# Lu-Zhan/Pano-NeRF

Hardware: AMD Instinct MI355X
Metric: rays/sec (train step) (higher is better)
Workload: dtype f32 (2xfp16 split products, fp32 accumulate; weight-gradient operands h_l / delta_l / r_l / hdot_l stored with 16 significant bits, 'Q24')

## Files before the change

### pano-nerf_amd/csrc/pn_chain.hip

```cpp
#include "pn_common.h"
#include <math.h>
#include <string.h>
#include <stdlib.h>
#include <type_traits>
#include <utility>
#include <vector>

template <typename F, int... Is>
__device__ __forceinline__ void static_for_impl(F&& f, std::integer_sequence<int, Is...>) {
    (f(std::integral_constant<int, Is>{}), ...);
}
template <int N, typename F>
__device__ __forceinline__ void static_for(F&& f) {
    static_for_impl(static_cast<F&&>(f), std::make_integer_sequence<int, N>{});
}

typedef __bf16 bf16x8 __attribute__((ext_vector_type(8)));
typedef _Float16 f16x8 __attribute__((ext_vector_type(8)));
typedef __attribute__((address_space(3))) void* lds_ptr_t;
typedef const __attribute__((address_space(1))) void* gbl_ptr_t;

#ifndef PN_CHAIN_TILE
#define PN_CHAIN_TILE 16
#endif
// ... 153 lines not shown
    constexpr int CF = Cfg<NP>::CF, SLOT = Cfg<NP>::SLOT, PER = Cfg<NP>::PER;
    const int64_t gid = (int64_t)blockIdx.x * blockDim.x + threadIdx.x;
    const int lane = (int)(gid & 63);
    const int64_t fi = gid >> 6;
    const int chunk = (int)(fi / (CF + 1)), f = (int)(fi % (CF + 1));
    if (chunk >= tab.nchunks) return;
    int li = 0;
    for (int i = 1; i < tab.n; ++i)
        if (chunk >= tab.L[i].chunk0) li = i;
    const PackLayer& L = tab.L[li];
    unsigned char* dst = out + (int64_t)chunk * SLOT + f * 1024 + lane * 16;
    if (f == CF) {
        float v[4] = {0.f, 0.f, 0.f, 0.f};
        if (chunk == L.chunk0 + (L.KS * L.NT + PER - 1) / PER - 1 && L.aux_off >= 0)
            for (int q = 0; q < 4; ++q)
                if (lane * 4 + q < L.aux_n) v[q] = params[L.aux_off + lane * 4 + q];
        memcpy(dst, v, 16);
        return;
    }
    const int p = f % NP;
    const int step = (chunk - L.chunk0) * PER + f / NP;
    int wex = 0;
    if constexpr (NP == 2) {
        const uint32_t* wm = reinterpret_cast<const uint32_t*>(wexp) + 32 + li * WEXP_SLICES;
        uint32_t top = 0u;
#pragma unroll
        for (int sl = 0; sl < WEXP_SLICES; ++sl) top = wm[sl] > top ? wm[sl] : top;
        wex = scale_exp(__uint_as_float(top), EXP_CAP_W);
        if (chunk == L.chunk0 && f == 0 && lane == 0) wexp[li] = wex;
    }
    unsigned short o[8] = {0, 0, 0, 0, 0, 0, 0, 0};
    if (step < L.KS * L.NT) {
        const int ks = step / L.NT, tt = step % L.NT;
        const int i = TILE * tt + (lane % TILE), g = lane / TILE;
        for (int j = 0; j < 8; ++j) {
            const int k = kmap(ks, g, j);
            float x = 0.f;
            if (i < L.rows_valid)
                for (int s = 0; s < L.nseg; ++s) {
                    const PackSeg& sg = L.seg[s];
                    const int kr = k - sg.k0;
                    if (kr >= 0 && kr < sg.kvalid)
                        x = sg.transposed ? params[sg.off + (int64_t)kr * sg.ld + sg.col0 + i]
                                          : params[sg.off + (int64_t)i * sg.ld + sg.col0 + kr];
                }
            unsigned short bits;
            if constexpr (NP == 2) {
                const float t = ldexpf(x, wex);
                const _Float16 hh = (_Float16)t;
                const _Float16 r = p == 0 ? hh : (_Float16)(t - (float)hh);
                __builtin_memcpy(&bits, &r, 2);
            } else {
                const __bf16 hb = (__bf16)x;
                __bf16 r = hb;
                if (p >= 1) {
                    const float r1 = x - (float)hb;
                    const __bf16 mb = (__bf16)r1;
                    r = mb;
                    if (p == 2) r = (__bf16)(r1 - (float)mb);
                }
                __builtin_memcpy(&bits, &r, 2);
            }
            o[j] = bits;
        }
    }
    memcpy(dst, o, 16);
}

#if defined(PN_TRACE_CHAIN) || defined(PN_TRACE_WG)
__device__ unsigned long long g_chain_trace[64];
extern "C" int pn_chain_trace_read(unsigned long long* out) {
    return hipMemcpyFromSymbol(out, HIP_SYMBOL(g_chain_trace), sizeof(unsigned long long) * 64) == hipSuccess ? 0 : -4;
}
#endif
#ifdef PN_TRACE_CHAIN
#define TR(i)                                                                                          \
    do {                                                                                               \
        if (blockIdx.x == 0 && threadIdx.x == 0 && st == (int64_t)gridDim.x) g_chain_trace[i] = __builtin_amdgcn_s_memtime(); \
    } while (0)
#define TRX(i)                                                                                 \
    do {                                                                                       \
        if (blockIdx.x == 0 && threadIdx.x == 0) g_chain_trace[i] = __builtin_amdgcn_s_memtime(); \
    } while (0)
#else
#define TR(i)
#define TRX(i)
#endif

template <int NP>
struct Ring {
    static constexpr int CF = Cfg<NP>::CF, SLOT = Cfg<NP>::SLOT;
    static constexpr int PIECES = CF / CH_WAVES + 1;
    __amdgpu_buffer_rsrc_t rsrc;
    unsigned char* lds;
    uint32_t lds_addr;
    int nchunk;
    int pf, pslot, cslot;
    int wid, lane;
    int cur_soff;
    unsigned char* cur_lds;
    __device__ __forceinline__ void begin_round() {
        cur_soff = pf * SLOT;
        cur_lds = lds + pslot * SLOT;
        pf = (pf + 1 == nchunk) ? 0 : pf + 1;
        pslot = (pslot + 1 == Cfg<NP>::NSLOT) ? 0 : pslot + 1;
    }
    template <int I, bool AUX>
    __device__ __forceinline__ void piece() {
        if constexpr (I < CF / CH_WAVES) {
            const int f = wid + CH_WAVES * I;
            __builtin_amdgcn_raw_ptr_buffer_load_lds(rsrc, (lds_ptr_t)(cur_lds + f * 1024), 16, lane * 16, cur_soff + f * 1024, 0, 0);
        } else if constexpr (I == CF / CH_WAVES && AUX) {
            if (wid < 4) {
                const int o = CF * 1024 + wid * 256;
                __builtin_amdgcn_raw_ptr_buffer_load_lds(rsrc, (lds_ptr_t)(cur_lds + o), 4, lane * 4, cur_soff + o, 0, 0);
            }
        }
    }
    template <int I0, int STRIDE, bool AUX = true>
    __device__ __forceinline__ void pieces_from() {
        if constexpr (I0 < PIECES) {
            piece<I0, AUX>();
            pieces_from<I0 + STRIDE, STRIDE, AUX>();
        }
    }
    __device__ __forceinline__ void start(const unsigned char* s, unsigned char* l, int n, int w, int ln, int first) {
        rsrc = __builtin_amdgcn_make_buffer_rsrc((void*)s, 0, n * SLOT, 0x00020000);
        lds = l; nchunk = n; wid = w; lane = ln;
        lds_addr = (uint32_t)(uintptr_t)(lds_ptr_t)l;
        pf = first; pslot = 0; cslot = 0;
#pragma unroll
        for (int i = 0; i < Cfg<NP>::D; ++i) {
            begin_round();
            pieces_from<0, 1, true>();
        }
    }
#ifdef PN_TRACE_CHAIN
    unsigned long long t_lds = 0, t_dma = 0, t_bar = 0, n_acq = 0;
#endif
    __device__ __forceinline__ uint32_t acquire() {
        constexpr int N = Cfg<NP>::SHARE * (Cfg<NP>::D - 1);
#ifdef PN_TRACE_CHAIN
        const unsigned long long t0 = __builtin_amdgcn_s_memtime();
        asm volatile("s_waitcnt lgkmcnt(0)" ::: "memory");
        const unsigned long long t1 = __builtin_amdgcn_s_memtime();
        asm volatile("s_waitcnt vmcnt(%0) lgkmcnt(0)" ::"n"(N) : "memory");
        const unsigned long long t2 = __builtin_amdgcn_s_memtime();
        __builtin_amdgcn_s_barrier();
        const unsigned long long t3 = __builtin_amdgcn_s_memtime();
        asm volatile("s_waitcnt lgkmcnt(0)" ::: "memory");
        t_lds += t1 - t0; t_dma += t2 - t1; t_bar += t3 - t2; ++n_acq;
#else
        asm volatile("s_waitcnt vmcnt(%0) lgkmcnt(0)" ::"n"(N) : "memory");
        if constexpr (!(PN_ABL_CHAIN & 8)) __builtin_amdgcn_s_barrier();
#endif
        begin_round();
        const uint32_t p = lds_addr + cslot * SLOT;
        cslot = (cslot + 1 == Cfg<NP>::NSLOT) ? 0 : cslot + 1;
        return p;
    }
    __device__ __forceinline__ void drain() {
        asm volatile("s_waitcnt vmcnt(0)" ::: "memory");
        __builtin_amdgcn_s_barrier();
#ifdef PN_TRACE_CHAIN
        if (blockIdx.x == 0 && threadIdx.x == 0) {
            g_chain_trace[56] = t_lds; g_chain_trace[57] = t_dma; g_chain_trace[58] = t_bar; g_chain_trace[59] = n_acq;
        }
#endif
    }
// ... 558 lines not shown
__device__ __forceinline__ Tile tile_of(int64_t st, int wid, int lane, int64_t M) {
    Tile t;
    t.c = lane % TILE;
    t.g = lane / TILE;
    t.blk = st * CH_WAVES + wid;
    t.row = t.blk * TILE + t.c;
    t.live = t.row < M;
    t.rc = t.live ? t.row : M - 1;
    t.lo = t.c + 4 * t.g * TILE;
    return t;
}
template <int NP, int NT>
__device__ __forceinline__ void store_vec(typename TEl<NP>::type* slot, const Tile& T, int F, bool q, const accv (&acc)[NT]) {
    if constexpr (kQ24<NP>) {
        if (q) {
            store_q24<NT>(reinterpret_cast<unsigned char*>(slot) + T.blk * (int64_t)(F * TILE * 3) + opaque(q24_lane(T.c, T.g)), acc);
            return;
        }
    }
    store_t<NT>(slot + T.blk * (int64_t)(F * TILE) + opaque(T.lo), acc);
}

template <int NP, int MODE>
__device__ __forceinline__ Ex encode(const float (&mu)[3], const float (&cv)[3], const float (&vv)[3], int g,
                                      typename TEl<NP>::type* et, BFrag<NP> (&benc)[KS_ENC]) {
    typedef typename TEl<NP>::type TE;
    constexpr int NQ = 96 / QB;
    float x[NQ][4];
    const int g4 = 4 * opaque(g);
#pragma unroll
    for (int qb = 0; qb < NQ / 2; ++qb)
#pragma unroll
        for (int i = 0; i < 4; ++i) {
            int l, ch;
            level_of(QB * qb + g4 + i, l, ch);
            const float sc = pow2i(l);
            const float y = sel3(mu, ch) * sc;
            const float e0 = __expf(-0.5f * (sel3(cv, ch) * (sc * sc)));
            if constexpr (MODE == 0) {
                x[qb][i] = e0 * fast_sin(y);
                x[qb + NQ / 2][i] = e0 * fast_sin(y + HALF_PI_F);
            } else {
                const float e = e0 * sc * sel3(vv, ch);
                x[qb][i] = e * fast_cos(y);
                x[qb + NQ / 2][i] = e * fast_cos(y + HALF_PI_F);
            }
        }
#ifdef PN_TRACE_CHAIN
#pragma unroll
    for (int qb = 0; qb < NQ; ++qb)
#pragma unroll
        for (int i = 0; i < 4; ++i) asm volatile("" ::"v"(x[qb][i]));
    if (MODE == 0) TRX(31);
#endif
#pragma unroll
    for (int qb = 0; qb < NQ; ++qb)
#pragma unroll
        for (int i = 0; i < 4; ++i) et[(QB * qb + i) * TILE] = (TE)x[qb][i];
    if (MODE == 0) TRX(32);
    Ex e{0, 0u};
    if constexpr (NP == 2) {
        if constexpr (MODE == 0) {
            e.ex = EXP_TOP - 1;
            e.top = 0x3f800000u;
        } else {
            float m = 0.f;
#pragma unroll
            for (int qb = 0; qb < NQ; ++qb)
#pragma unroll
                for (int i = 0; i < 4; ++i) m = fmaxf(m, fabsf(x[qb][i]));
            e = ex_of(m, EXP_CAP_Z);
        }
    }
#pragma unroll
    for (int s = 0; s < KS_ENC; ++s) {
        float y8[8];
#pragma unroll
        for (int j = 0; j < 8; ++j) y8[j] = x[2 * s + (j >> 2)][j & 3];
        split_into<NP>(y8, benc[s], e.ex);
    }
    return e;
}
template <int NP, int KS>
__device__ __forceinline__ int reload_b(const typename TEl<NP>::type* src, BFrag<NP> (&b)[KS], int cap = EXP_CAP) {
    if constexpr (NP == 2) {
        float x[KS][8];
        float m = 0.f;
#pragma unroll
        for (int ks = 0; ks < KS; ++ks)
#pragma unroll
            for (int j = 0; j < 8; ++j) {
                x[ks][j] = (float)src[(QB * (2 * ks + (j >> 2)) + (j & 3)) * TILE];
                m = fmaxf(m, fabsf(x[ks][j]));
            }
        const int ex = scale_exp(col_max(m), cap);
#pragma unroll
        for (int ks = 0; ks < KS; ++ks) split_into<NP>(x[ks], b[ks], ex);
        return ex;
    } else {
#pragma unroll
        for (int ks = 0; ks < KS; ++ks) {
            float x[8];
#pragma unroll
            for (int j = 0; j < 8; ++j) x[j] = (float)src[(QB * (2 * ks + (j >> 2)) + (j & 3)) * TILE];
            split_into<NP>(x, b[ks]);
        }
        return 0;
    }
}
__device__ __forceinline__ void ipe_backward_tiles(const accv (&acc)[NT_ENC], const float (&mu)[3], const float (&cv)[3], int g,
                                                   float (&dm)[3]) {
    dm[0] = dm[1] = dm[2] = 0.f;
    const int g4 = 4 * opaque(g);
#pragma unroll
    for (int qb = 0; qb < 96 / QB; ++qb)
#pragma unroll
        for (int i = 0; i < 4; ++i) {
            const bool cosine = qb >= 96 / QB / 2;
            int l, ch;
            level_of(QB * (cosine ? qb - 96 / QB / 2 : qb) + g4 + i, l, ch);
            const float sc = pow2i(l);
            const float y = sel3(mu, ch) * sc;
            const float ex = __expf(-0.5f * (sel3(cv, ch) * (sc * sc))) * sc;
            const float d = AQ(acc, qb, i) * ex * fast_cos(cosine ? y + HALF_PI_F : y);
            dm[0] += ch == 0 ? d : 0.f;
            dm[1] += ch == 1 ? d : 0.f;
            dm[2] += ch == 2 ? d : 0.f;
        }
#pragma unroll
    for (int i = 0; i < 3; ++i) {
        dm[i] = col_sum(dm[i]);
    }
}
template <int NP>
__device__ __forceinline__ Ex finish_gated(accv (&acc)[NT_H], const Gate& m, typename TEl<NP>::type* slot, const Tile& T, bool q24,
                                           BFrag<NP> (&bh)[KS_H]) {
    gate_bits<NT_H>(acc, m);
    if (slot) store_vec<NP, NT_H>(slot, T, 256, q24, acc);
    return acc_to_b<NP, NT_H, KS_H>(acc, bh, 0.f, EXP_CAP_Z);
}

__global__ void k_view_table(int64_t view_rows, const float* viewdirs, float* tab, uint32_t* amax, int amax_n) {
    if (amax && blockIdx.x == 0 && (int)threadIdx.x < amax_n) amax[threadIdx.x] = 0u;
    const int64_t idx = (int64_t)blockIdx.x * blockDim.x + threadIdx.x;
    if (idx >= view_rows * 32) return;
    const int64_t r = idx >> 5;
    const int v = (int)(idx & 31);
    const float vd0 = viewdirs[r * 3], vd1 = viewdirs[r * 3 + 1], vd2 = viewdirs[r * 3 + 2];
    auto vsel = [&](int ch) { return ch == 0 ? vd0 : (ch == 1 ? vd1 : vd2); };
    const int i = v - 3, half = i >= 12 ? 1 : 0;
    int l, ch;
    level_of(i < 0 ? 0 : i - 12 * half, l, ch);
    const float xb = vsel(ch) * pow2i(l & 3);
    const float sv = fast_sin(half ? xb + HALF_PI_F : xb);
    tab[idx] = v < 3 ? vsel(v) : (v < PN_VIEW_DIM ? sv : 0.f);
}

struct FwdArgs {
    int64_t M, nst;
    int rows_per_ray, nc;
    int64_t view_rows;
    const unsigned char* pack;
    const int* wexp;
    uint32_t* amax;
    const float* mean;
    const float* cov;
    const float* viewdirs;
    float* view_tab;
    float* enc_t;
    float* acts_t;
    uint32_t* masks;
    float* raw_rgb;
    float* raw_den;
    int q24;
};
__host__ __device__ constexpr int64_t act_off(int slot, int64_t Mp) {
    return slot <= 8 ? (int64_t)slot * Mp * 256 : 8 * Mp * 256 + Mp * 288;
}
__host__ __device__ constexpr int64_t acts_floats(int64_t Mp) { return 8 * Mp * 256 + Mp * 288 + Mp * 128; }

template <int NP>
__global__ __launch_bounds__(CH_THREADS, CH_MIN_WAVES) void k_chain_fwd(FwdArgs a) {
    extern __shared__ __attribute__((aligned(16))) unsigned char lds[];
    typedef typename TEl<NP>::type TE;
    const int tid = threadIdx.x, lane = tid & 63;
    const int wid = __builtin_amdgcn_readfirstlane(tid >> 6);
    const int64_t Mp = a.nst * CH_SAMPLES;
    chain_prio(wid);
    Ring<NP> R;
    R.start(a.pack, lds, fwd_chunk0<NP>(F_COUNT), wid, lane, 0);
    RunMax<10> RM;
    RM.clear();
#ifdef PN_TRACE_CHAIN
    if (blockIdx.x == 0 && threadIdx.x == 0) {
        g_chain_trace[60] = __builtin_amdgcn_s_memtime();
        g_chain_trace[61] = __builtin_amdgcn_s_memrealtime();
    }
#endif
    int wtab = 0;
    if constexpr (NP == 2) wtab = a.wexp[lane & 15];
    for (int64_t st = blockIdx.x; st < a.nst; st += gridDim.x) {
        const Tile T = tile_of(st, wid, lane, a.M);
        TR(0);
        TE* et = TP(a.enc_t) + T.blk * (96 * TILE) + T.lo;
        BFrag<NP> bh[KS_H];
        accv acc[NT_H];
        Gate mw;
        int bex = 0;
        auto wx = [&](int i) {
            if constexpr (NP == 2) return __builtin_amdgcn_readlane(wtab, i);
            else return 0;
        };
        {
            float mu[3], cv[3];
            const float zero3[3] = {0.f, 0.f, 0.f};
#pragma unroll
            for (int i = 0; i < 3; ++i) {
                mu[i] = a.mean[T.rc * 3 + i];
                cv[i] = a.cov[T.rc * 3 + i];
            }
            BFrag<NP> benc[KS_ENC];
#ifdef PN_TRACE_CHAIN
            asm volatile("" ::"v"(mu[0]), "v"(mu[1]), "v"(mu[2]), "v"(cv[0]), "v"(cv[1]), "v"(cv[2]));
            TRX(30);
#endif
            bex = encode<NP, 0>(mu, cv, zero3, T.g, et, benc).ex;
            TR(1);
            chain_gemm<NP, KS_ENC, NT_H, true, true, true>(R, benc, acc, lane, wx(F_L0) + bex);
            TR(2);
        }
        auto finish_hidden = [&](int slot) {
            relu<NT_H>(acc);
            if (TP(a.acts_t)) store_vec<NP, NT_H>(TP(a.acts_t) + act_off(slot, Mp), T, 256, a.q24 && q24_act(slot), acc);
            const Ex e = acc_to_b<NP, NT_H, KS_H>(acc, bh);
            gate_words<NP, KS_H, KS_H>(bh, mw);
            store_gate(a.masks, slot, Mp, T.blk * TILE + T.c, T.g, mw);
            bex = e.ex;
            RM.upd(slot, e.top);
        };
        finish_hidden(0);
        TR(3);
#pragma unroll 1
        for (int l = 1; l <= 4; ++l) {
            chain_gemm<NP, KS_H, NT_H, true, true, true>(R, bh, acc, lane, wx(F_L0 + l) + bex);
            TR(2 + 2 * l);
            finish_hidden(l);
            TR(3 + 2 * l);
        }
        {
            chain_gemm<NP, KS_H, NT_H, false, true, true>(R, bh, acc, lane, wx(F_L5) + bex);
            BFrag<NP> benc[KS_ENC];
            const int eex = reload_b<NP, KS_ENC>(et, benc);
            chain_gemm<NP, KS_ENC, NT_H, true, false, true>(R, benc, acc, lane, wx(F_L5E) + eex);
            TR(12);
            finish_hidden(5);
            TR(13);
        }
#pragma unroll 1
        for (int l = 6; l <= 7; ++l) {
            chain_gemm<NP, KS_H, NT_H, true, true, true>(R, bh, acc, lane, wx(F_L6 + l - 6) + bex);
            TR(2 + 2 * l);
            finish_hidden(l);
            TR(3 + 2 * l);
        }
        {
            accv ad[1];
            chain_gemm<NP, KS_H, 1, true, true, true>(R, bh, ad, lane, wx(F_DEN) + bex);
            if (T.live) {
#pragma unroll
                for (int i = 0; i < 4; ++i) {
                    const int ch = 4 * T.g + i;
                    if (ch < a.nc) a.raw_den[T.row * a.nc + ch] = ad[0][i];
                }
            }
        }
        TR(18);
        BFrag<NP> bv[KS_H + KS_PAD];
        int vex;
        {
            chain_gemm<NP, KS_H, NT_H, true, true, true>(R, bh, acc, lane, wx(F_EXTRA) + bex);
            TR(19);
            TE* bt = a.acts_t ? TP(a.acts_t) + act_off(8, Mp) + T.blk * (288 * TILE) + T.lo : nullptr;
            if (bt) store_t<NT_H>(bt, acc);
            const Ex e = acc_to_b<NP, NT_H, KS_H + KS_PAD>(acc, bv, 1.0f);
            vex = e.ex;
            RM.upd(8, e.top);
            const float* vt = a.view_tab + ((T.rc / a.rows_per_ray) % a.view_rows) * 32 + 4 * T.g;
#pragma unroll
            for (int q = 0; q < KS_PAD; ++q) {
                float x[8];
#pragma unroll
                for (int h = 0; h < 2; ++h) {
                    const f32x4 v = *reinterpret_cast<const f32x4*>(vt + QB * (2 * q + h));
#pragma unroll
                    for (int i = 0; i < 4; ++i) {
                        x[4 * h + i] = v[i];
                        if (bt) bt[(256 + QB * (2 * q + h) + i) * TILE] = (TE)v[i];
                    }
                }
                split_into<NP>(x, bv[KS_H + q], vex);
            }
        }
        TR(20);
        BFrag<NP> bc[KS_C];
        int cex;
        {
            accv av[NT_C];
            chain_gemm<NP, KS_H + KS_PAD, NT_C, true, true, true>(R, bv, av, lane, wx(F_VIEW) + vex);
            TR(21);
            Gate w4;
            relu<NT_C>(av);
            if (TP(a.acts_t)) store_t<NT_C>(TP(a.acts_t) + act_off(9, Mp) + T.blk * (128 * TILE) + T.lo, av);
            const Ex e = acc_to_b<NP, NT_C, KS_C>(av, bc);
            gate_words<NP, KS_C, KS_C>(bc, w4);
            store_gate(a.masks, 8, Mp, T.blk * TILE + T.c, T.g, w4);
            cex = e.ex;
            RM.upd(9, e.top);
        }
        TR(22);
        {
            accv ac[1];
            chain_gemm<NP, KS_C, 1, true, true, true>(R, bc, ac, lane, wx(F_COLOR) + cex);
            TR(23);
            if (T.live && T.g == 0) {
#pragma unroll
                for (int e = 0; e < 3; ++e) a.raw_rgb[T.row * 3 + e] = ac[0][e];
            }
        }
        TR(24);
    }
    R.drain();
#ifdef PN_TRACE_CHAIN
    if (blockIdx.x == 0 && threadIdx.x == 0) {
        g_chain_trace[62] = __builtin_amdgcn_s_memtime();
        g_chain_trace[63] = __builtin_amdgcn_s_memrealtime();
    }
#endif
    if constexpr (NP == 2) {
        RM.flush(a.amax ? a.amax + AM_ACT0 : nullptr, lane, wid, lds);
        if (a.amax && blockIdx.x == 0 && tid == 0) a.amax[AM_ENC] = 0x3f800000u;
    }
}

struct SweepArgs {
    int64_t M, nst;
    int nc;
    float density_bias;
    const unsigned char* pack;
    int nchunk;
    const int* wexp;
    uint32_t* amax;
    const uint32_t* masks;
    const float* raw_den;
    const float* mean;
    const float* cov;
    const float* wd0;
    const float* v;
    float* vec_t;
    int keep_all;
    float* edot_t;
    float* out3;
    float* sdot;
    int q24;
};

template <int NP>
__global__ __launch_bounds__(CH_THREADS, CH_MIN_WAVES) void k_chain_dgrad(SweepArgs a) {
    extern __shared__ __attribute__((aligned(16))) unsigned char lds[];
    typedef typename TEl<NP>::type TE;
    const int tid = threadIdx.x, lane = tid & 63;
    const int wid = __builtin_amdgcn_readfirstlane(tid >> 6);
    const int64_t Mp = a.nst * CH_SAMPLES;
    chain_prio(wid);
    Ring<NP> R;
    R.start(a.pack, lds, a.nchunk, wid, lane, 0);
    RunMax<8> RM;
    RM.clear();
    int wtab = 0;
    if constexpr (NP == 2) wtab = a.wexp[lane & 15];
    for (int64_t st = blockIdx.x; st < a.nst; st += gridDim.x) {
        const Tile T = tile_of(st, wid, lane, a.M);
        Gate mk[8];
#pragma unroll
        for (int l = 0; l < 8; ++l) mk[l] = load_gate(a.masks, 7 - l, Mp, T.blk * TILE + T.c, T.g);
        float mu[3], cv[3];
#pragma unroll
        for (int i = 0; i < 3; ++i) {
            mu[i] = a.mean[T.rc * 3 + i];
            cv[i] = a.cov[T.rc * 3 + i];
        }
        const float sgm = T.live ? ch_sp_d1(a.raw_den[T.rc * a.nc] + a.density_bias) : 0.f;
        BFrag<NP> bh[KS_H];
        int bex = 0;
        auto wx = [&](int i) {
            if constexpr (NP == 2) return __builtin_amdgcn_readlane(wtab, i);
            else return 0;
        };
        {
            const bool Q7 = kQ24<NP> && a.q24 && q24_delta(7);
            TE* rt = (a.keep_all && !Q7) ? TP(a.vec_t) + (int64_t)7 * Mp * 256 + T.blk * (256 * TILE) + T.lo : nullptr;
            unsigned char* rq = (a.keep_all && Q7) ? reinterpret_cast<unsigned char*>(TP(a.vec_t) + (int64_t)7 * Mp * 256) +
                                                         T.blk * (int64_t)(256 * TILE * 3) + q24_lane(T.c, T.g)
                                                   : nullptr;
            const Gate m7 = pop_front(mk);
            if constexpr (NP == 2) {
                float wm = 0.f;
#pragma unroll
                for (int qb = 0; qb < NT_H * ACCQ; ++qb) {
                    const f32x4 wv = *reinterpret_cast<const f32x4*>(a.wd0 + QB * qb + 4 * T.g);
                    wm = fmaxf(fmaxf(wm, fmaxf(fabsf(wv[0]), fabsf(wv[1]))), fmaxf(fabsf(wv[2]), fabsf(wv[3])));
                }
                const Ex e = ex_of(sgm * wm, EXP_CAP_Z);
                bex = e.ex;
                RM.upd(7, e.top);
            }
#pragma unroll
            for (int ks = 0; ks < KS_H; ++ks) {
                float x[8];
#pragma unroll
                for (int h = 0; h < 2; ++h) {
                    const f32x4 wv = *reinterpret_cast<const f32x4*>(a.wd0 + QB * (2 * ks + h) + 4 * T.g);
#pragma unroll
                    for (int i = 0; i < 4; ++i) {
                        const int j = 4 * h + i;
                        const uint32_t bit = (m7.w[gate_word(ks, j)] >> gate_bit(ks, j)) & 1u;
                        x[j] = bit ? sgm * wv[i] : 0.f;
                        if (rt) rt[(QB * (2 * ks + h) + i) * TILE] = (TE)x[j];
                    }
                    if constexpr (kQ24<NP>) {
                        if (rq) {
#if PN_Q24_NT
                            __builtin_nontemporal_store(pack_q24(x[4 * h], x[4 * h + 1], x[4 * h + 2], x[4 * h + 3]), reinterpret_cast<u32x3*>(rq + (2 * ks + h) * 768));
#else
                            *reinterpret_cast<u32x3*>(rq + (2 * ks + h) * 768) = pack_q24(x[4 * h], x[4 * h + 1], x[4 * h + 2], x[4 * h + 3]);
#endif
                        }
                    }
                }
                split_into<NP>(x, bh[ks], bex);
            }
        }
        accv acc[NT_H];
#pragma unroll 1
        for (int l = 7; l >= 1; --l) {
            chain_gemm<NP, KS_H, NT_H, false, true>(R, bh, acc, lane, wx(B_L7 + 7 - l) + bex);
            TE* dst = a.keep_all ? TP(a.vec_t) + (int64_t)(l - 1) * Mp * 256 : (l - 1 == 5 ? TP(a.vec_t) : nullptr);
            const Ex e = finish_gated<NP>(acc, pop_front(mk), dst, T, a.q24 && q24_delta(l - 1), bh);
            bex = e.ex;
            RM.upd(l - 1, e.top);
        }
        {
            accv a3[NT_ENC];
            chain_gemm<NP, KS_H, NT_ENC, false, true>(R, bh, a3, lane, wx(B_DENC0) + bex);
            bex = reload_b<NP, KS_H>(TP(a.vec_t) + (a.keep_all ? (int64_t)5 * Mp * 256 : 0) + T.blk * (256 * TILE) + T.lo, bh, EXP_CAP_Z);
            chain_gemm<NP, KS_H, NT_ENC, false, false>(R, bh, a3, lane, wx(B_DENC1) + bex);
            float dm[3];
            ipe_backward_tiles(a3, mu, cv, T.g, dm);
            if (T.live && T.g == 0) {
                a.out3[T.row * 3] = dm[0];
                a.out3[T.row * 3 + 1] = dm[1];
                a.out3[T.row * 3 + 2] = dm[2];
            }
        }
    }
    R.drain();
    if constexpr (NP == 2) RM.flush(a.amax ? a.amax + AM_RS0 : nullptr, lane, wid, lds);
}

template <int NP>
__global__ __launch_bounds__(CH_THREADS, CH_MIN_WAVES) void k_chain_tangent(SweepArgs a) {
    extern __shared__ __attribute__((aligned(16))) unsigned char lds[];
    typedef typename TEl<NP>::type TE;
    const int tid = threadIdx.x, lane = tid & 63;
    const int wid = __builtin_amdgcn_readfirstlane(tid >> 6);
    const int64_t Mp = a.nst * CH_SAMPLES;
    chain_prio(wid);
    Ring<NP> R;
    R.start(a.pack, lds, a.nchunk, wid, lane, 0);
    RunMax<9> RM;
    RM.clear();
    Ex e;
    int wtab = 0;
    if constexpr (NP == 2) wtab = a.wexp[lane & 15];
    for (int64_t st = blockIdx.x; st < a.nst; st += gridDim.x) {
        const Tile T = tile_of(st, wid, lane, a.M);
        Gate mk[8];
#pragma unroll
        for (int l = 0; l < 8; ++l) mk[l] = load_gate(a.masks, l, Mp, T.blk * TILE + T.c, T.g);
        TE* et = TP(a.edot_t) + T.blk * (96 * TILE) + T.lo;
        BFrag<NP> bh[KS_H];
        accv acc[NT_H];
        int bex = 0;
        auto wx = [&](int i) {
            if constexpr (NP == 2) return __builtin_amdgcn_readlane(wtab, i);
            else return 0;
        };
        {
            float mu[3], cv[3], vv[3];
#pragma unroll
            for (int i = 0; i < 3; ++i) {
                mu[i] = a.mean[T.rc * 3 + i];
                cv[i] = a.cov[T.rc * 3 + i];
                vv[i] = T.live ? a.v[T.rc * 3 + i] : 0.f;
            }
            BFrag<NP> benc[KS_ENC];
            e = encode<NP, 1>(mu, cv, vv, T.g, et, benc);
            bex = e.ex;
            RM.upd(8, e.top);
            chain_gemm<NP, KS_ENC, NT_H, false, true>(R, benc, acc, lane, wx(F_L0) + bex);
        }
        e = finish_gated<NP>(acc, pop_front(mk), TP(a.vec_t), T, a.q24 && q24_act(0), bh);
        bex = e.ex;
        RM.upd(0, e.top);
#pragma unroll 1
        for (int l = 1; l <= 4; ++l) {
            chain_gemm<NP, KS_H, NT_H, false, true>(R, bh, acc, lane, wx(F_L0 + l) + bex);
            e = finish_gated<NP>(acc, pop_front(mk), TP(a.vec_t) + (int64_t)l * Mp * 256, T, a.q24 && q24_act(l), bh);
            bex = e.ex;
            RM.upd(l, e.top);
        }
        {
            chain_gemm<NP, KS_H, NT_H, false, true>(R, bh, acc, lane, wx(F_L5) + bex);
            BFrag<NP> benc[KS_ENC];
            const int eex = reload_b<NP, KS_ENC>(et, benc, EXP_CAP_Z);
            chain_gemm<NP, KS_ENC, NT_H, false, false>(R, benc, acc, lane, wx(F_L5E) + eex);
            e = finish_gated<NP>(acc, pop_front(mk), TP(a.vec_t) + (int64_t)5 * Mp * 256, T, a.q24 && q24_act(5), bh);
            bex = e.ex;
            RM.upd(5, e.top);
        }
        chain_gemm<NP, KS_H, NT_H, false, true>(R, bh, acc, lane, wx(F_L6) + bex);
        e = finish_gated<NP>(acc, pop_front(mk), TP(a.vec_t) + (int64_t)6 * Mp * 256, T, a.q24 && q24_act(6), bh);
        bex = e.ex;
        RM.upd(6, e.top);
        chain_gemm<NP, KS_H, NT_H, false, true>(R, bh, acc, lane, wx(F_L7) + bex);
        {
            gate_bits<NT_H>(acc, pop_front(mk));
            store_t<NT_H>(TP(a.vec_t) + (int64_t)7 * Mp * 256 + T.blk * (256 * TILE) + T.lo, acc);
            if constexpr (NP == 2) RM.upd(7, ex_of(lane_amax<NT_H>(acc), EXP_CAP_Z).top);
            float sd = 0.f;
#pragma unroll
            for (int qb = 0; qb < NT_H * ACCQ; ++qb) {
                const f32x4 wv = *reinterpret_cast<const f32x4*>(a.wd0 + QB * qb + 4 * T.g);
#pragma unroll
                for (int i = 0; i < 4; ++i) sd += AQ(acc, qb, i) * wv[i];
            }
            sd = col_sum(sd);
            if (T.live && T.g == 0) a.sdot[T.row] = sd;
        }
    }
    R.drain();
    if constexpr (NP == 2) RM.flush(a.amax ? a.amax + AM_TANG0 : nullptr, lane, wid, lds);
}

struct BwdArgs {
    int64_t M, nst;
    int nc;
    float density_bias;
    const unsigned char* pack;
    int nchunk;
    const int* wexp;
    uint32_t* amax;
    const uint32_t* masks;
    const float* raw_den;
    const float* d_rgb;
    const float* d_den;
    const float* sdot;
    const float* mean;
    const float* cov;
    float* drgb_t;
    float* dhv_t;
    float* d8_t;
    float* delta_t;
    float* coef_t;
    float* d_mean;
    int q24;
};

template <int NP>
__global__ __launch_bounds__(CH_THREADS, CH_MIN_WAVES) void k_chain_bwd(BwdArgs a) {
    extern __shared__ __attribute__((aligned(16))) unsigned char lds[];
    typedef typename TEl<NP>::type TE;
    const int tid = threadIdx.x, lane = tid & 63;
    const int wid = __builtin_amdgcn_readfirstlane(tid >> 6);
    const int64_t Mp = a.nst * CH_SAMPLES;
    chain_prio(wid);
    Ring<NP> R;
    R.start(a.pack, lds, a.nchunk, wid, lane, 0);
    RunMax<12> RM;
    RM.clear();
    Ex e;
    int wtab = 0;
    if constexpr (NP == 2) wtab = a.wexp[lane & 15];
    for (int64_t st = blockIdx.x; st < a.nst; st += gridDim.x) {
        const Tile T = tile_of(st, wid, lane, a.M);
        Gate mk[9];
#pragma unroll
        for (int l = 0; l < 9; ++l) mk[l] = load_gate(a.masks, 8 - l, Mp, T.blk * TILE + T.c, T.g);
        BFrag<NP> b1[1];
        int bex = 0;
        auto wx = [&](int i) {
            if constexpr (NP == 2) return __builtin_amdgcn_readlane(wtab, i);
            else return 0;
        };
        {
            float x[8];
            TE* dt = TP(a.drgb_t) + T.blk * (32 * TILE) + T.lo;
            float m = 0.f;
#pragma unroll
            for (int j = 0; j < 8; ++j) {
                const int f = QB * (j >> 2) + 4 * T.g + (j & 3);
                x[j] = (T.live && f < 3) ? a.d_rgb[T.rc * 3 + (f < 3 ? f : 0)] : 0.f;
                dt[(QB * (j >> 2) + (j & 3)) * TILE] = (TE)x[j];
                m = fmaxf(m, fabsf(x[j]));
            }
            if constexpr (NP == 2) {
                e = ex_of(m, EXP_CAP_Z);
                bex = e.ex;
                RM.upd(11, e.top);
            }
            split_into<NP>(x, b1[0], bex);
        }
        BFrag<NP> bc[KS_C];
        {
            accv av[NT_C];
            chain_gemm<NP, 1, NT_C, false, true>(R, b1, av, lane, wx(B_COLOR) + bex);
            gate_bits<NT_C>(av, pop_front(mk));
            store_t<NT_C>(TP(a.dhv_t) + T.blk * (128 * TILE) + T.lo, av);
            e = acc_to_b<NP, NT_C, KS_C>(av, bc, 0.f, EXP_CAP_Z);
            bex = e.ex;
            RM.upd(10, e.top);
        }
        BFrag<NP> be[KS_H + 1];
        accv acc[NT_H];
        {
            chain_gemm<NP, KS_C, NT_H, false, true>(R, bc, acc, lane, wx(B_VIEW) + bex);
            TE* bt = TP(a.d8_t) + T.blk * (288 * TILE) + T.lo;
            store_t<NT_H>(bt, acc);
            const float z = a.raw_den[T.rc * a.nc] + a.density_bias;
            const float add0 = (a.sdot && T.live) ? ch_sp_d2(z) * a.sdot[T.rc] : 0.f;
            float x[8];
            float m = 0.f;
#pragma unroll
            for (int j = 0; j < 8; ++j) {
                const int ch = QB * (j >> 2) + 4 * T.g + (j & 3);
                float v = 0.f;
                if (T.live && ch < a.nc) v = a.d_den[T.rc * a.nc + ch] + (ch == 0 ? add0 : 0.f);
                x[j] = v;
                bt[(256 + QB * (j >> 2) + (j & 3)) * TILE] = (TE)v;
                m = fmaxf(m, fabsf(v));
            }
            if constexpr (NP == 2) {
                e = ex_of(lane_amax<NT_H>(acc), EXP_CAP_Z);
                const Ex ed = ex_of(m, EXP_CAP_Z);
                RM.upd(8, e.top);
                RM.upd(9, ed.top);
                bex = e.ex < ed.ex ? e.ex : ed.ex;
            }
            split_acc<NP, NT_H, KS_H + 1>(acc, be, bex);
            split_into<NP>(x, be[KS_H], bex);
            if (TP(a.coef_t)) {
                TE* ct = TP(a.coef_t) + T.blk * (32 * TILE) + T.lo;
                const float cf = T.live ? ch_sp_d1(z) : 0.f;
#pragma unroll
                for (int j = 0; j < 8; ++j) {
                    const int f = QB * (j >> 2) + 4 * T.g + (j & 3);
                    ct[(QB * (j >> 2) + (j & 3)) * TILE] = (TE)(f == 0 ? cf : 0.f);
                }
            }
        }
        BFrag<NP> bh[KS_H];
        chain_gemm<NP, KS_H + 1, NT_H, false, true>(R, be, acc, lane, wx(B_EXTRA) + bex);
        e = finish_gated<NP>(acc, pop_front(mk), TP(a.delta_t) + (int64_t)7 * Mp * 256, T, a.q24 && q24_delta(7), bh);
        bex = e.ex;
        RM.upd(7, e.top);
#pragma unroll 1
        for (int l = 7; l >= 1; --l) {
            chain_gemm<NP, KS_H, NT_H, false, true>(R, bh, acc, lane, wx(B_L7 + 7 - l) + bex);
            e = finish_gated<NP>(acc, pop_front(mk), TP(a.delta_t) + (int64_t)(l - 1) * Mp * 256, T, a.q24 && q24_delta(l - 1), bh);
            bex = e.ex;
            RM.upd(l - 1, e.top);
        }
        if (a.d_mean) {
            float mu[3], cv[3];
#pragma unroll
            for (int i = 0; i < 3; ++i) {
                mu[i] = a.mean[T.rc * 3 + i];
                cv[i] = a.cov[T.rc * 3 + i];
            }
            accv a3[NT_ENC];
            chain_gemm<NP, KS_H, NT_ENC, false, true>(R, bh, a3, lane, wx(B_DENC0) + bex);
            bex = reload_b<NP, KS_H>(TP(a.delta_t) + (int64_t)5 * Mp * 256 + T.blk * (256 * TILE) + T.lo, bh, EXP_CAP_Z);
            chain_gemm<NP, KS_H, NT_ENC, false, false>(R, bh, a3, lane, wx(B_DENC1) + bex);
            float dm[3];
            ipe_backward_tiles(a3, mu, cv, T.g, dm);
            if (T.live && T.g == 0) {
                a.d_mean[T.row * 3] = dm[0];
                a.d_mean[T.row * 3 + 1] = dm[1];
                a.d_mean[T.row * 3 + 2] = dm[2];
            }
        }
    }
    R.drain();
    if constexpr (NP == 2) {
        RM.flush(a.amax ? a.amax + AM_DELTA0 : nullptr, lane, wid, lds);
        if (a.amax && blockIdx.x == 0 && tid == 0) a.amax[AM_COEF] = 0x3f800000u;
    }
}

struct WSeg {
    const float* X;
    const float* Y;
    int64_t nhalf;
    int FX, FY;
    int bias;
    const uint32_t* ax;
    const uint32_t* ay;
};
struct WgArgs {
    WSeg seg[4];
    int nseg;
    int64_t half_total, per;
    float* slab;
    int64_t slab_stride;
    int bias;
};
constexpr int WG_MAXJ = 8;
struct WgMulti {
    WgArgs job[WG_MAXJ];
};

template <int NP>
__device__ __forceinline__ f32x16 mfma_split32(const BFrag<NP>& a, const BFrag<NP>& b, f32x16 v) {
    if constexpr (NP == 3) {
        v = __builtin_amdgcn_mfma_f32_32x32x16_bf16(a.p[2], b.p[0], v, 0, 0, 0);
        v = __builtin_amdgcn_mfma_f32_32x32x16_bf16(a.p[0], b.p[2], v, 0, 0, 0);
        v = __builtin_amdgcn_mfma_f32_32x32x16_bf16(a.p[1], b.p[1], v, 0, 0, 0);
        v = __builtin_amdgcn_mfma_f32_32x32x16_bf16(a.p[1], b.p[0], v, 0, 0, 0);
        v = __builtin_amdgcn_mfma_f32_32x32x16_bf16(a.p[0], b.p[1], v, 0, 0, 0);
        v = __builtin_amdgcn_mfma_f32_32x32x16_bf16(a.p[0], b.p[0], v, 0, 0, 0);
    } else if constexpr (NP == 2) {
        v = __builtin_amdgcn_mfma_f32_32x32x16_f16(a.p[1], b.p[0], v, 0, 0, 0);
        v = __builtin_amdgcn_mfma_f32_32x32x16_f16(a.p[0], b.p[1], v, 0, 0, 0);
        v = __builtin_amdgcn_mfma_f32_32x32x16_f16(a.p[0], b.p[0], v, 0, 0, 0);
    } else {
        v = __builtin_amdgcn_mfma_f32_32x32x16_bf16(a.p[0], b.p[0], v, 0, 0, 0);
    }
    return v;
}
#define WG_LD(p) __builtin_nontemporal_load(p)
#ifndef PN_WG_UNIT_NT
#define PN_WG_UNIT_NT 0
#endif
#if PN_WG_UNIT_NT
#define WG_LDU(p) __builtin_nontemporal_load(p)
#else
#define WG_LDU(p) (*(p))
#endif
template <int NP, int TM, int TN, int WM, int WN, bool X24 = false, bool Y24 = false>
__global__ __launch_bounds__(64 * WM * WN) void k_chain_wgrad(WgMulti multi) {
    const WgArgs& a = multi.job[blockIdx.y];
    static_assert(!(X24 || Y24) || (NP == 2 && TILE == 16), "Q24 tensors exist in fp16-pair builds with 16-sample tiles");
    static_assert(!X24 || Y24, "combinations in use: (0,0), (0,1), (1,1)");
    constexpr bool ROT = X24 || Y24;
    constexpr int NTH = 64 * WM * WN, TMW = 32 * TM * WM, TNW = 32 * TN * WN;
    constexpr int PX = TMW * 16, PY = TNW * 16;
    constexpr int BUF = NP * (PX + PY);
    typedef typename TEl<NP>::type TE;
    constexpr int PPR = 16 * (int)sizeof(TE) / 16;
    constexpr int SPP = 16 / PPR;
    constexpr int CX = X24 ? 0 : TMW * PPR, CY = Y24 ? 0 : TNW * PPR;
    constexpr int LX = X24 ? 1 : (CX + NTH - 1) / NTH, LY = Y24 ? 1 : (CY + NTH - 1) / NTH;
    constexpr int UX = X24 ? TMW : 0, UY = Y24 ? TNW : 0;
    constexpr int LU = (UX + UY + NTH - 1) / NTH;
    static_assert(UX % 64 == 0, "a wave's units are all X or all Y");
#ifndef PN_WG_UNIT_COAL
#define PN_WG_UNIT_COAL 0
#endif
    constexpr bool COAL = PN_WG_UNIT_COAL && (X24 || Y24);
    constexpr int SCR = COAL ? (NTH / 64) * 1536 : 0;
    __shared__ __attribute__((aligned(16))) unsigned short smem[2 * BUF + SCR];
    const int tid = threadIdx.x, lane = tid & 63;
    const int wid = __builtin_amdgcn_readfirstlane(tid >> 6);
    const int wm = wid / WN, wn = wid % WN;
// ... 1114 lines not shown
```

Measured before the change: 186,400.

## Prefetch next tile's backward inputs and split reload loads from conversion

In the backward chain kernel, the per-tile scalar inputs (gate, d_rgb, raw density, sdot, d_den) are now loaded for the next tile during the current tile's last GEMM stages, so their latency is hidden behind work. Gate masks are loaded one layer at a time rather than all nine upfront, which lowers register pressure. The activation reload is split into a load phase and a split phase, and in bwd the load is issued before the preceding GEMM. The view-table loads are hoisted into a batch. It also adds trace points that compile away by default, at the cost of more live registers across the loop and more complex control flow.

```diff
diff --git a/pano-nerf_amd/csrc/pn_chain.hip b/pano-nerf_amd/csrc/pn_chain.hip
--- a/pano-nerf_amd/csrc/pn_chain.hip
+++ b/pano-nerf_amd/csrc/pn_chain.hip
@@ -259,9 +259,23 @@
     do {                                                                                       \
         if (blockIdx.x == 0 && threadIdx.x == 0) g_chain_trace[i] = __builtin_amdgcn_s_memtime(); \
     } while (0)
+template <typename A>
+__device__ __forceinline__ void tr_landed1(const A& x) {
+    asm volatile("" ::"v"(x));
+}
+template <typename... A>
+__device__ __forceinline__ void tr_landed(const A&... x) {
+    (tr_landed1(x), ...);
+}
+#define TRW(i, ...)              \
+    do {                         \
+        tr_landed(__VA_ARGS__);  \
+        TR(i);                   \
+    } while (0)
 #else
 #define TR(i)
 #define TRX(i)
+#define TRW(i, ...)
 #endif
 
 template <int NP>
@@ -986,31 +1000,36 @@
     return e;
 }
 template <int NP, int KS>
-__device__ __forceinline__ int reload_b(const typename TEl<NP>::type* src, BFrag<NP> (&b)[KS], int cap = EXP_CAP) {
+struct Reload {
+    typename TEl<NP>::type x[KS][8];
+};
+template <int NP, int KS>
+__device__ __forceinline__ void reload_load(const typename TEl<NP>::type* src, Reload<NP, KS>& r) {
+#pragma unroll
+    for (int ks = 0; ks < KS; ++ks)
+#pragma unroll
+        for (int j = 0; j < 8; ++j) r.x[ks][j] = src[(QB * (2 * ks + (j >> 2)) + (j & 3)) * TILE];
+}
+template <int NP, int KS>
+__device__ __forceinline__ int reload_split(const Reload<NP, KS>& r, BFrag<NP> (&b)[KS], int cap = EXP_CAP) {
+    int ex = 0;
     if constexpr (NP == 2) {
-        float x[KS][8];
         float m = 0.f;
 #pragma unroll
         for (int ks = 0; ks < KS; ++ks)
 #pragma unroll
-            for (int j = 0; j < 8; ++j) {
-                x[ks][j] = (float)src[(QB * (2 * ks + (j >> 2)) + (j & 3)) * TILE];
-                m = fmaxf(m, fabsf(x[ks][j]));
-            }
-        const int ex = scale_exp(col_max(m), cap);
-#pragma unroll
-        for (int ks = 0; ks < KS; ++ks) split_into<NP>(x[ks], b[ks], ex);
-        return ex;
-    } else {
-#pragma unroll
-        for (int ks = 0; ks < KS; ++ks) {
-            float x[8];
-#pragma unroll
-            for (int j = 0; j < 8; ++j) x[j] = (float)src[(QB * (2 * ks + (j >> 2)) + (j & 3)) * TILE];
-            split_into<NP>(x, b[ks]);
-        }
-        return 0;
-    }
+            for (int j = 0; j < 8; ++j) m = fmaxf(m, fabsf((float)r.x[ks][j]));
+        ex = scale_exp(col_max(m), cap);
+    }
+#pragma unroll
+    for (int ks = 0; ks < KS; ++ks) {
+        float x[8];
+#pragma unroll
+        for (int j = 0; j < 8; ++j) x[j] = (float)r.x[ks][j];
+        if constexpr (NP == 2) split_into<NP>(x, b[ks], ex);
+        else split_into<NP>(x, b[ks]);
+    }
+    return ex;
 }
 __device__ __forceinline__ void ipe_backward_tiles(const accv (&acc)[NT_ENC], const float (&mu)[3], const float (&cv)[3], int g,
                                                    float (&dm)[3]) {
@@ -1106,6 +1125,7 @@
     for (int64_t st = blockIdx.x; st < a.nst; st += gridDim.x) {
         const Tile T = tile_of(st, wid, lane, a.M);
         TR(0);
+        TR(33);
         TE* et = TP(a.enc_t) + T.blk * (96 * TILE) + T.lo;
         BFrag<NP> bh[KS_H];
         accv acc[NT_H];
@@ -1127,6 +1147,7 @@
 #ifdef PN_TRACE_CHAIN
             asm volatile("" ::"v"(mu[0]), "v"(mu[1]), "v"(mu[2]), "v"(cv[0]), "v"(cv[1]), "v"(cv[2]));
             TRX(30);
+            TR(34);
 #endif
             bex = encode<NP, 0>(mu, cv, zero3, T.g, et, benc).ex;
             TR(1);
@@ -1154,7 +1175,11 @@
         {
             chain_gemm<NP, KS_H, NT_H, false, true, true>(R, bh, acc, lane, wx(F_L5) + bex);
             BFrag<NP> benc[KS_ENC];
-            const int eex = reload_b<NP, KS_ENC>(et, benc);
+            Reload<NP, KS_ENC> re;
+            TR(37);
+            reload_load<NP, KS_ENC>(et, re);
+            TRW(38, (float)re.x[0][0], (float)re.x[KS_ENC - 1][7]);
+            const int eex = reload_split<NP, KS_ENC>(re, benc);
             chain_gemm<NP, KS_ENC, NT_H, true, false, true>(R, benc, acc, lane, wx(F_L5E) + eex);
             TR(12);
             finish_hidden(5);
@@ -1190,12 +1215,17 @@
             vex = e.ex;
             RM.upd(8, e.top);
             const float* vt = a.view_tab + ((T.rc / a.rows_per_ray) % a.view_rows) * 32 + 4 * T.g;
+            TR(35);
+            f32x4 vw[2 * KS_PAD];
+#pragma unroll
+            for (int i = 0; i < 2 * KS_PAD; ++i) vw[i] = *reinterpret_cast<const f32x4*>(vt + QB * i);
+            TRW(36, vw[0], vw[2 * KS_PAD - 1]);
 #pragma unroll
             for (int q = 0; q < KS_PAD; ++q) {
                 float x[8];
 #pragma unroll
                 for (int h = 0; h < 2; ++h) {
-                    const f32x4 v = *reinterpret_cast<const f32x4*>(vt + QB * (2 * q + h));
+                    const f32x4 v = vw[2 * q + h];
 #pragma unroll
                     for (int i = 0; i < 4; ++i) {
                         x[4 * h + i] = v[i];
@@ -1232,6 +1262,7 @@
             }
         }
         TR(24);
+        TR(39);
     }
     R.drain();
 #ifdef PN_TRACE_CHAIN
@@ -1285,6 +1316,7 @@
     for (int64_t st = blockIdx.x; st < a.nst; st += gridDim.x) {
         const Tile T = tile_of(st, wid, lane, a.M);
         Gate mk[8];
+        TR(33);
 #pragma unroll
         for (int l = 0; l < 8; ++l) mk[l] = load_gate(a.masks, 7 - l, Mp, T.blk * TILE + T.c, T.g);
         float mu[3], cv[3];
@@ -1293,7 +1325,9 @@
             mu[i] = a.mean[T.rc * 3 + i];
             cv[i] = a.cov[T.rc * 3 + i];
         }
-        const float sgm = T.live ? ch_sp_d1(a.raw_den[T.rc * a.nc] + a.density_bias) : 0.f;
+        const float rd0 = a.raw_den[T.rc * a.nc];
+        TRW(34, mk[0].w[0], mk[7].w[MW - 1], mu[0], mu[2], cv[0], cv[2], rd0);
+        const float sgm = T.live ? ch_sp_d1(rd0 + a.density_bias) : 0.f;
         BFrag<NP> bh[KS_H];
         int bex = 0;
         auto wx = [&](int i) {
@@ -1356,7 +1390,11 @@
         {
             accv a3[NT_ENC];
             chain_gemm<NP, KS_H, NT_ENC, false, true>(R, bh, a3, lane, wx(B_DENC0) + bex);
-            bex = reload_b<NP, KS_H>(TP(a.vec_t) + (a.keep_all ? (int64_t)5 * Mp * 256 : 0) + T.blk * (256 * TILE) + T.lo, bh, EXP_CAP_Z);
+            Reload<NP, KS_H> r5;
+            TR(37);
+            reload_load<NP, KS_H>(TP(a.vec_t) + (a.keep_all ? (int64_t)5 * Mp * 256 : 0) + T.blk * (256 * TILE) + T.lo, r5);
+            TRW(38, (float)r5.x[0][0], (float)r5.x[KS_H - 1][7]);
+            bex = reload_split<NP, KS_H>(r5, bh, EXP_CAP_Z);
             chain_gemm<NP, KS_H, NT_ENC, false, false>(R, bh, a3, lane, wx(B_DENC1) + bex);
             float dm[3];
             ipe_backward_tiles(a3, mu, cv, T.g, dm);
@@ -1366,6 +1404,7 @@
                 a.out3[T.row * 3 + 2] = dm[2];
             }
         }
+        TR(39);
     }
     R.drain();
     if constexpr (NP == 2) RM.flush(a.amax ? a.amax + AM_RS0 : nullptr, lane, wid, lds);
@@ -1389,6 +1428,7 @@
     for (int64_t st = blockIdx.x; st < a.nst; st += gridDim.x) {
         const Tile T = tile_of(st, wid, lane, a.M);
         Gate mk[8];
+        TR(33);
 #pragma unroll
         for (int l = 0; l < 8; ++l) mk[l] = load_gate(a.masks, l, Mp, T.blk * TILE + T.c, T.g);
         TE* et = TP(a.edot_t) + T.blk * (96 * TILE) + T.lo;
@@ -1407,6 +1447,7 @@
                 cv[i] = a.cov[T.rc * 3 + i];
                 vv[i] = T.live ? a.v[T.rc * 3 + i] : 0.f;
             }
+            TRW(34, mk[0].w[0], mk[7].w[MW - 1], mu[0], mu[2], cv[0], cv[2], vv[0], vv[2]);
             BFrag<NP> benc[KS_ENC];
             e = encode<NP, 1>(mu, cv, vv, T.g, et, benc);
             bex = e.ex;
@@ -1426,7 +1467,11 @@
         {
             chain_gemm<NP, KS_H, NT_H, false, true>(R, bh, acc, lane, wx(F_L5) + bex);
             BFrag<NP> benc[KS_ENC];
-            const int eex = reload_b<NP, KS_ENC>(et, benc, EXP_CAP_Z);
+            Reload<NP, KS_ENC> re;
+            TR(37);
+            reload_load<NP, KS_ENC>(et, re);
+            TRW(38, (float)re.x[0][0], (float)re.x[KS_ENC - 1][7]);
+            const int eex = reload_split<NP, KS_ENC>(re, benc, EXP_CAP_Z);
             chain_gemm<NP, KS_ENC, NT_H, false, false>(R, benc, acc, lane, wx(F_L5E) + eex);
             e = finish_gated<NP>(acc, pop_front(mk), TP(a.vec_t) + (int64_t)5 * Mp * 256, T, a.q24 && q24_act(5), bh);
             bex = e.ex;
@@ -1451,6 +1496,7 @@
             sd = col_sum(sd);
             if (T.live && T.g == 0) a.sdot[T.row] = sd;
         }
+        TR(39);
     }
     R.drain();
     if constexpr (NP == 2) RM.flush(a.amax ? a.amax + AM_TANG0 : nullptr, lane, wid, lds);
@@ -1480,6 +1526,23 @@
     int q24;
 };
 
+struct BwdIn {
+    Gate gv;
+    float drgb[3];
+    float rd0, sdot;
+    float dden[4];
+};
+__device__ __forceinline__ void tile_inputs(const BwdArgs& a, int64_t st, int wid, int lane, int64_t Mp, BwdIn& in) {
+    const Tile T = tile_of(st, wid, lane, a.M);
+    in.gv = load_gate(a.masks, 8, Mp, T.blk * TILE + T.c, T.g);
+#pragma unroll
+    for (int j = 0; j < 3; ++j) in.drgb[j] = (T.live && T.g == 0) ? a.d_rgb[T.rc * 3 + j] : 0.f;
+    in.rd0 = a.raw_den[T.rc * a.nc];
+    in.sdot = (a.sdot && T.live) ? a.sdot[T.rc] : 0.f;
+#pragma unroll
+    for (int j = 0; j < 4; ++j) in.dden[j] = (T.live && 4 * T.g + j < a.nc) ? a.d_den[T.rc * a.nc + 4 * T.g + j] : 0.f;
+}
+
 template <int NP>
 __global__ __launch_bounds__(CH_THREADS, CH_MIN_WAVES) void k_chain_bwd(BwdArgs a) {
     extern __shared__ __attribute__((aligned(16))) unsigned char lds[];
@@ -1488,6 +1551,8 @@
     const int wid = __builtin_amdgcn_readfirstlane(tid >> 6);
     const int64_t Mp = a.nst * CH_SAMPLES;
     chain_prio(wid);
+    BwdIn in;
+    if ((int64_t)blockIdx.x < a.nst) tile_inputs(a, blockIdx.x, wid, lane, Mp, in);
     Ring<NP> R;
     R.start(a.pack, lds, a.nchunk, wid, lane, 0);
     RunMax<12> RM;
@@ -1497,9 +1562,8 @@
     if constexpr (NP == 2) wtab = a.wexp[lane & 15];
     for (int64_t st = blockIdx.x; st < a.nst; st += gridDim.x) {
         const Tile T = tile_of(st, wid, lane, a.M);
-        Gate mk[9];
-#pragma unroll
-        for (int l = 0; l < 9; ++l) mk[l] = load_gate(a.masks, 8 - l, Mp, T.blk * TILE + T.c, T.g);
+        auto gate_of = [&](int slot) { return load_gate(a.masks, slot, Mp, T.blk * TILE + T.c, T.g); };
+        TR(33);
         BFrag<NP> b1[1];
         int bex = 0;
         auto wx = [&](int i) {
@@ -1512,11 +1576,11 @@
             float m = 0.f;
 #pragma unroll
             for (int j = 0; j < 8; ++j) {
-                const int f = QB * (j >> 2) + 4 * T.g + (j & 3);
-                x[j] = (T.live && f < 3) ? a.d_rgb[T.rc * 3 + (f < 3 ? f : 0)] : 0.f;
+                x[j] = j < 3 ? in.drgb[j] : 0.f;
                 dt[(QB * (j >> 2) + (j & 3)) * TILE] = (TE)x[j];
                 m = fmaxf(m, fabsf(x[j]));
             }
+            TRW(34, in.gv.w[0], x[0], x[1], x[2]);
             if constexpr (NP == 2) {
                 e = ex_of(m, EXP_CAP_Z);
                 bex = e.ex;
@@ -1528,7 +1592,7 @@
         {
             accv av[NT_C];
             chain_gemm<NP, 1, NT_C, false, true>(R, b1, av, lane, wx(B_COLOR) + bex);
-            gate_bits<NT_C>(av, pop_front(mk));
+            gate_bits<NT_C>(av, in.gv);
             store_t<NT_C>(TP(a.dhv_t) + T.blk * (128 * TILE) + T.lo, av);
             e = acc_to_b<NP, NT_C, KS_C>(av, bc, 0.f, EXP_CAP_Z);
             bex = e.ex;
@@ -1538,21 +1602,23 @@
         accv acc[NT_H];
         {
             chain_gemm<NP, KS_C, NT_H, false, true>(R, bc, acc, lane, wx(B_VIEW) + bex);
-            TE* bt = TP(a.d8_t) + T.blk * (288 * TILE) + T.lo;
+            TE* bt = TP(a.d8_t) + T.blk * (288 * TILE) + opaque(T.lo);
             store_t<NT_H>(bt, acc);
-            const float z = a.raw_den[T.rc * a.nc] + a.density_bias;
-            const float add0 = (a.sdot && T.live) ? ch_sp_d2(z) * a.sdot[T.rc] : 0.f;
+            TR(35);
+            const float z = in.rd0 + a.density_bias;
+            const float add0 = (a.sdot && T.live) ? ch_sp_d2(z) * in.sdot : 0.f;
             float x[8];
             float m = 0.f;
 #pragma unroll
             for (int j = 0; j < 8; ++j) {
                 const int ch = QB * (j >> 2) + 4 * T.g + (j & 3);
                 float v = 0.f;
-                if (T.live && ch < a.nc) v = a.d_den[T.rc * a.nc + ch] + (ch == 0 ? add0 : 0.f);
+                if (j < 4 && T.live && ch < a.nc) v = in.dden[j & 3] + (ch == 0 ? add0 : 0.f);
                 x[j] = v;
                 bt[(256 + QB * (j >> 2) + (j & 3)) * TILE] = (TE)v;
                 m = fmaxf(m, fabsf(v));
             }
+            TRW(36, z, add0, x[0], x[1], x[2], x[3], x[4], x[5], x[6], x[7]);
             if constexpr (NP == 2) {
                 e = ex_of(lane_amax<NT_H>(acc), EXP_CAP_Z);
                 const Ex ed = ex_of(m, EXP_CAP_Z);
@@ -1563,7 +1629,7 @@
             split_acc<NP, NT_H, KS_H + 1>(acc, be, bex);
             split_into<NP>(x, be[KS_H], bex);
             if (TP(a.coef_t)) {
-                TE* ct = TP(a.coef_t) + T.blk * (32 * TILE) + T.lo;
+                TE* ct = TP(a.coef_t) + T.blk * (32 * TILE) + opaque(T.lo);
                 const float cf = T.live ? ch_sp_d1(z) : 0.f;
 #pragma unroll
                 for (int j = 0; j < 8; ++j) {
@@ -1573,14 +1639,17 @@
             }
         }
         BFrag<NP> bh[KS_H];
+        const Gate g7 = gate_of(7);
         chain_gemm<NP, KS_H + 1, NT_H, false, true>(R, be, acc, lane, wx(B_EXTRA) + bex);
-        e = finish_gated<NP>(acc, pop_front(mk), TP(a.delta_t) + (int64_t)7 * Mp * 256, T, a.q24 && q24_delta(7), bh);
+        e = finish_gated<NP>(acc, g7, TP(a.delta_t) + (int64_t)7 * Mp * 256, T, a.q24 && q24_delta(7), bh);
         bex = e.ex;
         RM.upd(7, e.top);
 #pragma unroll 1
         for (int l = 7; l >= 1; --l) {
+            const Gate gl = gate_of(l - 1);
+            if (l == 1 && !a.d_mean && st + gridDim.x < a.nst) tile_inputs(a, st + gridDim.x, wid, lane, Mp, in);
             chain_gemm<NP, KS_H, NT_H, false, true>(R, bh, acc, lane, wx(B_L7 + 7 - l) + bex);
-            e = finish_gated<NP>(acc, pop_front(mk), TP(a.delta_t) + (int64_t)(l - 1) * Mp * 256, T, a.q24 && q24_delta(l - 1), bh);
+            e = finish_gated<NP>(acc, gl, TP(a.delta_t) + (int64_t)(l - 1) * Mp * 256, T, a.q24 && q24_delta(l - 1), bh);
             bex = e.ex;
             RM.upd(l - 1, e.top);
         }
@@ -1591,9 +1660,14 @@
                 mu[i] = a.mean[T.rc * 3 + i];
                 cv[i] = a.cov[T.rc * 3 + i];
             }
+            Reload<NP, KS_H> r5;
+            reload_load<NP, KS_H>(TP(a.delta_t) + (int64_t)5 * Mp * 256 + T.blk * (256 * TILE) + opaque(T.lo), r5);
             accv a3[NT_ENC];
             chain_gemm<NP, KS_H, NT_ENC, false, true>(R, bh, a3, lane, wx(B_DENC0) + bex);
-            bex = reload_b<NP, KS_H>(TP(a.delta_t) + (int64_t)5 * Mp * 256 + T.blk * (256 * TILE) + T.lo, bh, EXP_CAP_Z);
+            TR(37);
+            TRW(38, (float)r5.x[0][0], (float)r5.x[KS_H - 1][7]);
+            bex = reload_split<NP, KS_H>(r5, bh, EXP_CAP_Z);
+            if (st + gridDim.x < a.nst) tile_inputs(a, st + gridDim.x, wid, lane, Mp, in);
             chain_gemm<NP, KS_H, NT_ENC, false, false>(R, bh, a3, lane, wx(B_DENC1) + bex);
             float dm[3];
             ipe_backward_tiles(a3, mu, cv, T.g, dm);
@@ -1603,6 +1677,7 @@
                 a.d_mean[T.row * 3 + 2] = dm[2];
             }
         }
+        TR(39);
     }
     R.drain();
     if constexpr (NP == 2) {
```

After: 185,800. Within noise of the previous version (-0.3%).
